# kdsuneraavinash/CH-Bin

Hardware: NVIDIA B200
Metric: point-to-hull QP distances/sec (higher is better)
Workload: dtype f64

## Files before the change

### ch-bin_b200/csrc/fused.cu

```cuda
#include <cuda.h>

#include <algorithm>
#include <cmath>
#include <cstdlib>

#include "common.cuh"

namespace {

constexpr int BM = 128, BN = 128, BK = 32;
constexpr int UMMA_K = 8;
constexpr uint32_t TILE_BYTES = BM * BK * 4;
constexpr int FUSED_THREADS = 320;
constexpr int EPI_THREADS = 256;
constexpr uint32_t TMEM_COLS = 256;
constexpr int MAX_BOX = 10;
constexpr int SMEM_LIMIT = 232448;
constexpr int DMAX_F = CHB_FUSED_RESIDENT_DMAX;
constexpr int DMAX_W = 1024;
constexpr int NKT_STREAMED = -1;
constexpr int WIDE_STAGE_BOXES = 4;

constexpr int NC = 16;
struct SmemTail {
    alignas(16) float cand_val[NC][EPI_THREADS];
    alignas(8) uint64_t full_bar[8];
    alignas(8) uint64_t empty_bar[8];
    alignas(8) uint64_t tmem_full_bar[2];
    alignas(8) uint64_t tmem_empty_bar[2];
    alignas(8) uint64_t a_full_bar;
    alignas(8) uint64_t a_empty_bar;
    alignas(8) uint2 prog[MAX_BOX * 8];
    int prog_start[MAX_BOX + 1];
    uint32_t tmem_base;
};

__device__ __forceinline__ uint32_t smem_u32(const void *p) { return (uint32_t)__cvta_generic_to_shared(p); }
__device__ __forceinline__ void st_shared_f32(uint32_t addr, float v) { asm volatile("st.shared.f32 [%0], %1;" ::"r"(addr), "f"(v) : "memory"); }
__device__ __forceinline__ float ld_shared_f32(uint32_t addr)
{
    float v;
    asm volatile("ld.shared.f32 %0, [%1];" : "=f"(v) : "r"(addr) : "memory");
    return v;
}
__device__ __forceinline__ void mbar_init(uint64_t *bar, uint32_t count)
{
    asm volatile("mbarrier.init.shared::cta.b64 [%0], %1;" ::"r"(smem_u32(bar)), "r"(count));
}
__device__ __forceinline__ void mbar_expect_tx(uint64_t *bar, uint32_t bytes)
{
    asm volatile("mbarrier.arrive.expect_tx.shared::cta.b64 _, [%0], %1;" ::"r"(smem_u32(bar)), "r"(bytes) : "memory");
}
__device__ __forceinline__ void mbar_arrive(uint64_t *bar)
{
    asm volatile("mbarrier.arrive.shared::cta.b64 _, [%0];" ::"r"(smem_u32(bar)) : "memory");
}
__device__ __forceinline__ void mbar_wait(uint64_t *bar, uint32_t parity)
{
    asm volatile(
        "{\n"
        ".reg .pred p;\n"
        "WAIT_LOOP:\n"
        "mbarrier.try_wait.parity.shared::cta.b64 p, [%0], %1;\n"
        "@p bra WAIT_DONE;\n"
        "bra WAIT_LOOP;\n"
        "WAIT_DONE:\n"
        "}\n" ::"r"(smem_u32(bar)),
        "r"(parity)
        : "memory");
}
__device__ __forceinline__ void tma_load_2d(void *smem_dst, const CUtensorMap *map, uint64_t *bar, int c0, int c1)
{
    asm volatile("cp.async.bulk.tensor.2d.shared::cluster.global.mbarrier::complete_tx::bytes [%0], [%1, {%3, %4}], [%2];"
                 ::"r"(smem_u32(smem_dst)), "l"(map), "r"(smem_u32(bar)), "r"(c0), "r"(c1)
                 : "memory");
}
__device__ __forceinline__ void umma_tf32(uint32_t tmem_d, uint64_t adesc, uint64_t bdesc, uint32_t idesc, uint32_t accumulate)
{
    asm volatile(
        "{\n"
        ".reg .pred p;\n"
        "setp.ne.b32 p, %4, 0;\n"
        "tcgen05.mma.cta_group::1.kind::tf32 [%0], %1, %2, %3, p;\n"
        "}\n" ::"r"(tmem_d),
        "l"(adesc), "l"(bdesc), "r"(idesc), "r"(accumulate)
        : "memory");
}
__device__ __forceinline__ bool elect_one_sync()
{
    uint32_t pred;
    asm volatile(
        "{\n"
        ".reg .pred P;\n"
        "elect.sync _|P, 0xffffffff;\n"
        "selp.b32 %0, 1, 0, P;\n"
        "}\n"
        : "=r"(pred));
    return pred != 0;
}
__device__ __forceinline__ void umma_commit(uint64_t *bar)
{
    asm volatile("tcgen05.commit.cta_group::1.mbarrier::arrive::one.shared::cluster.b64 [%0];" ::"r"(smem_u32(bar)) : "memory");
}

__global__ void round_reset_kernel(int32_t *__restrict__ bin_cnt, int32_t nbin_cnt, float *__restrict__ ym2, int32_t nym2,
                                   int32_t *__restrict__ row_nb, int64_t nown, int32_t *__restrict__ pair_meta, int32_t nmeta,
                                   int32_t *__restrict__ pair_row, int64_t cap_pairs, int32_t *__restrict__ counters,
                                   int64_t ncol, int32_t *__restrict__ col_pt, int32_t *__restrict__ col_a, int32_t *__restrict__ col_b)
{
    chb_pdl_enter();
    const int64_t i = (int64_t)blockIdx.x * blockDim.x + threadIdx.x;
    if (i < ncol) {
        col_pt[i] = -1;
        col_a[i] = INT32_MAX;
        col_b[i] = INT32_MIN;
    }
    if (i < nbin_cnt) bin_cnt[i] = 0;
    if (i < nym2) ym2[i] = 0.f;
    if (i < nown) row_nb[i] = 0;
    if (i < nmeta) pair_meta[i] = 0;
    if (i < cap_pairs) pair_row[i] = -1;
    if (i == 0) {
        counters[0] = 0; counters[6] = 0; counters[7] = 0; counters[8] = 0; counters[12] = 0; counters[14] = 0;
        counters[1] = 0x7f7f7f7f; counters[2] = 0; counters[3] = 0;
    }
}
// ... 760 lines not shown
            const int v = beg[b];
            nxt = v > nxt ? nxt : v;
            beg[b] = nxt;
        }
        totals[0] = TT;
    }
    if (beg_smem) {
        __syncthreads();
        for (int b = tid; b <= G; b += 1024) cta_begin[b] = s_begin[b];
    }
}

template <bool WIDE>
__global__ void __launch_bounds__(256) pairs_fill_kernel(const int32_t *__restrict__ mode, const int32_t *__restrict__ row_nb,
                                                         const int32_t *__restrict__ row_bins, int64_t nown, int32_t C,
                                                         const int32_t *__restrict__ pair_off, int32_t *__restrict__ pair_row,
                                                         int32_t *__restrict__ row_pid, const float *__restrict__ a2, int32_t Kp2,
                                                         float *__restrict__ ap)
{
    chb_pdl_enter();
    if (*mode != 1) return;
    const int lane = threadIdx.x & 31;
    const int64_t r = ((int64_t)blockIdx.x * blockDim.x + threadIdx.x) >> 5;
    if (r >= nown) return;
    const int nb = row_nb[r];
    if (nb == 0) return;
    const float4 *src = reinterpret_cast<const float4 *>(a2 + r * Kp2);
    const int nq = Kp2 / 4;
    float4 v[3];
    if constexpr (!WIDE) {
#pragma unroll
        for (int u = 0; u < 3; ++u) v[u] = (lane + 32 * u < nq) ? __ldg(src + lane + 32 * u) : make_float4(0.f, 0.f, 0.f, 0.f);
    }
    for (int jb = 0; jb < nb; jb += 32) {
        const int j = jb + lane;
        int id = -1;
        if (j < nb) {
            const int c = row_bins[r * C + j];
            id = pair_off[c] + row_pid[r * C + j];
            pair_row[id] = (int32_t)r;
            row_pid[r * C + j] = id;
        }
        const int cnt = nb - jb < 32 ? nb - jb : 32;
        for (int w = 0; w < cnt; ++w) {
            const int idw = __shfl_sync(CHB_FULL, id, w);
            float4 *dst = reinterpret_cast<float4 *>(ap + (int64_t)idw * Kp2);
            if constexpr (WIDE) {
                for (int u = lane; u < nq; u += 32) dst[u] = __ldg(src + u);
            } else {
#pragma unroll
                for (int u = 0; u < 3; ++u)
                    if (lane + 32 * u < nq) dst[lane + 32 * u] = v[u];
            }
        }
    }
}

template <int KR>
struct TopList {
    float key[KR];
    int idx[KR];
    __device__ __forceinline__ void reset()
    {
#pragma unroll
        for (int s = 0; s < KR; ++s) { key[s] = INFINITY; idx[s] = INT32_MAX; }
    }
    __device__ __forceinline__ void insert(float ka, int ki)
    {
        int cnt = 0;
#pragma unroll
        for (int s = 0; s < KR; ++s) cnt += (key[s] <= ka) ? 1 : 0;
#pragma unroll
        for (int s = KR - 1; s >= 1; --s) {
            const bool shift = s > cnt, here = s == cnt;
            key[s] = shift ? key[s - 1] : (here ? ka : key[s]);
            idx[s] = shift ? idx[s - 1] : (here ? ki : idx[s]);
        }
        key[0] = cnt == 0 ? ka : key[0];
        idx[0] = cnt == 0 ? ki : idx[0];
    }
};

template <int KR, int NKT>
__global__ void __launch_bounds__(FUSED_THREADS, 1)
gram_select_kernel(const __grid_constant__ CUtensorMap map_a, const __grid_constant__ CUtensorMap map_ap,
                   const __grid_constant__ CUtensorMap map_b, const int32_t *__restrict__ mode_p,
                   const int32_t *__restrict__ pair_row, int nbox, int nk, int nstage,
                   const int32_t *__restrict__ col_pt,
                   const int32_t *__restrict__ col_a, const int32_t *__restrict__ col_b, const float *__restrict__ col_nrm,
                   const float *__restrict__ tq_tab, const int32_t *__restrict__ row_point, const int32_t *__restrict__ pos,
                   int64_t nrows, int32_t C, const float *__restrict__ t0_tab, int64_t ldt, const int4 *__restrict__ items,
                   const int32_t *__restrict__ cta_begin, float *__restrict__ cand_key, int32_t *__restrict__ cand_idx,
                   int32_t *__restrict__ tiles_issued)
{
    chb_pdl_wait();
    const int item_begin = cta_begin[blockIdx.x], item_end = cta_begin[blockIdx.x + 1];
    const int mode = *mode_p;
    constexpr bool STREAM = NKT == NKT_STREAMED;
    constexpr uint32_t STAGE_BYTES = STREAM ? WIDE_STAGE_BOXES * TILE_BYTES : TILE_BYTES;
    extern __shared__ uint8_t smem_raw[];
    uint8_t *base = reinterpret_cast<uint8_t *>((reinterpret_cast<uintptr_t>(smem_raw) + 1023) & ~uintptr_t(1023));
    uint8_t *a_res = base;
    uint8_t *ring = STREAM ? base : base + (size_t)nbox * TILE_BYTES;
    SmemTail &S = *reinterpret_cast<SmemTail *>(ring + (size_t)nstage * STAGE_BYTES);
    const int warp = threadIdx.x >> 5, lane = threadIdx.x & 31;

    if (threadIdx.x == 0) {
        for (int s = 0; s < nstage; ++s) {
            mbar_init(&S.full_bar[s], 1);
            mbar_init(&S.empty_bar[s], 1);
        }
        for (int b = 0; b < 2; ++b) {
            mbar_init(&S.tmem_full_bar[b], 1);
            mbar_init(&S.tmem_empty_bar[b], 8);
        }
        mbar_init(&S.a_full_bar, 1);
        mbar_init(&S.a_empty_bar, 1);
        asm volatile("fence.mbarrier_init.release.cluster;" ::: "memory");
        asm volatile("prefetch.tensormap [%0];" ::"l"(&map_a) : "memory");
        asm volatile("prefetch.tensormap [%0];" ::"l"(&map_ap) : "memory");
        asm volatile("prefetch.tensormap [%0];" ::"l"(&map_b) : "memory");
    }
    if (warp == 2) {
        asm volatile("tcgen05.alloc.cta_group::1.sync.aligned.shared::cta.b32 [%0], %1;" ::"r"(smem_u32(&S.tmem_base)), "n"(TMEM_COLS));
        asm volatile("tcgen05.relinquish_alloc_permit.cta_group::1.sync.aligned;");
    }
    asm volatile("tcgen05.fence::before_thread_sync;" ::: "memory");
    __syncthreads();
    asm volatile("tcgen05.fence::after_thread_sync;" ::: "memory");
    const uint32_t tmem_base = S.tmem_base;

    if (warp == 0) {
        if (lane == 0) {
            int s = 0;
            uint32_t ph = 0;
            int cur_rb = -1, na = 0;
            for (int it = item_begin; it < item_end; ++it) {
                const int4 item = items[it];
                if constexpr (STREAM) {
                    const int H = nbox >> 1;
                    const CUtensorMap *mq = mode ? &map_ap : &map_a;
                    for (int t = item.z; t < item.z + item.w; ++t) {
                        for (int b = 0; b < H; ++b) {
                            uint8_t *st = ring + (size_t)s * STAGE_BYTES;
                            mbar_wait(&S.empty_bar[s], ph ^ 1);
                            mbar_expect_tx(&S.full_bar[s], STAGE_BYTES);
                            tma_load_2d(st, mq, &S.full_bar[s], b * BK, item.x * BM);
                            tma_load_2d(st + TILE_BYTES, mq, &S.full_bar[s], (H + b) * BK, item.x * BM);
                            tma_load_2d(st + 2 * TILE_BYTES, &map_b, &S.full_bar[s], b * BK, t * BN);
                            tma_load_2d(st + 3 * TILE_BYTES, &map_b, &S.full_bar[s], (H + b) * BK, t * BN);
                            if (++s == nstage) { s = 0; ph ^= 1; }
                        }
                    }
                    continue;
                }
                if (item.x != cur_rb) {
                    mbar_wait(&S.a_empty_bar, (uint32_t)((na & 1) ^ 1));
                    mbar_expect_tx(&S.a_full_bar, (uint32_t)nbox * TILE_BYTES);
                    for (int jb = 0; jb < nbox; ++jb)
                        tma_load_2d(a_res + (size_t)jb * TILE_BYTES, mode ? &map_ap : &map_a, &S.a_full_bar, jb * BK, item.x * BM);
                    cur_rb = item.x;
                    ++na;
                }
                for (int t = item.z; t < item.z + item.w; ++t) {
                    for (int jb = 0; jb < nbox; ++jb) {
                        mbar_wait(&S.empty_bar[s], ph ^ 1);
                        mbar_expect_tx(&S.full_bar[s], TILE_BYTES);
                        tma_load_2d(ring + (size_t)s * TILE_BYTES, &map_b, &S.full_bar[s], jb * BK, t * BN);
                        if (++s == nstage) { s = 0; ph ^= 1; }
                    }
                }
            }
        }
    } else if (warp == 1) {
        {
            const uint32_t idesc = (1u << 4) | (2u << 7) | (2u << 10) | ((uint32_t)(BN >> 3) << 17) | ((uint32_t)(BM >> 4) << 24);
            const uint32_t a_addr = smem_u32(a_res);
            constexpr uint32_t DESC_HI = (1024u >> 4) | (1u << 14) | (2u << 29);
            if (NKT == 0 && lane == 0) {
                int m = 0;
                for (int jb = 0; jb < nbox; ++jb) {
                    S.prog_start[jb] = m;
                    for (int u = 0; u < BK / UMMA_K; ++u) {
                        const int j = jb * (BK / UMMA_K) + u;
                        if (j >= 2 * nk) break;
                        const int i0 = j < nk ? j : j - nk;
                        const uint32_t boff = (uint32_t)((u * UMMA_K * 4) >> 4);
                        S.prog[m++] = make_uint2((((a_addr + (uint32_t)(i0 >> 2) * TILE_BYTES) & 0x3FFFFu) >> 4 | (1u << 16)) +
                                                     (uint32_t)(((i0 & 3) * UMMA_K * 4) >> 4), boff);
                        if (j < nk) {
                            const int i1 = nk + j;
                            S.prog[m++] = make_uint2((((a_addr + (uint32_t)(i1 >> 2) * TILE_BYTES) & 0x3FFFFu) >> 4 | (1u << 16)) +
                                                         (uint32_t)(((i1 & 3) * UMMA_K * 4) >> 4), boff);
                        }
                    }
                }
                S.prog_start[nbox] = m;
            }
            __syncwarp();
            const uint32_t ring_lo = ((smem_u32(ring) & 0x3FFFFu) >> 4) | (1u << 16);
            int s = 0;
            uint32_t ph = 0;
            int64_t tt = 0;
            int cur_rb = -1, na = 0;
            for (int it = item_begin; it < item_end; ++it) {
                const int4 item = items[it];
                if (!STREAM && item.x != cur_rb) {
                    if (cur_rb >= 0 && elect_one_sync()) umma_commit(&S.a_empty_bar);
                    mbar_wait(&S.a_full_bar, (uint32_t)(na & 1));
                    asm volatile("tcgen05.fence::after_thread_sync;" ::: "memory");
                    cur_rb = item.x;
                    ++na;
                }
                for (int t = item.z; t < item.z + item.w; ++t) {
                    const int buf = (int)(tt & 1);
                    const uint32_t tph = (uint32_t)((tt >> 1) & 1);
                    ++tt;
                    mbar_wait(&S.tmem_empty_bar[buf], tph ^ 1);
                    asm volatile("tcgen05.fence::after_thread_sync;" ::: "memory");
                    const uint32_t tmem_d = tmem_base + (uint32_t)(buf * BN);
                    if constexpr (STREAM) {
                        const int H = nbox >> 1;
                        for (int b = 0; b < H; ++b) {
                            const uint32_t st_lo = ring_lo + (uint32_t)s * (STAGE_BYTES >> 4);
                            mbar_wait(&S.full_bar[s], ph);
                            asm volatile("tcgen05.fence::after_thread_sync;" ::: "memory");
                            if (elect_one_sync()) {
#pragma unroll
                                for (int u = 0; u < BK / UMMA_K; ++u) {
                                    const uint32_t ko = (uint32_t)((u * UMMA_K * 4) >> 4);
                                    const uint64_t qhi = ((uint64_t)DESC_HI << 32) | (st_lo + ko);
                                    const uint64_t qlo = ((uint64_t)DESC_HI << 32) | (st_lo + (TILE_BYTES >> 4) + ko);
                                    const uint64_t chi = ((uint64_t)DESC_HI << 32) | (st_lo + 2 * (TILE_BYTES >> 4) + ko);
                                    const uint64_t clo = ((uint64_t)DESC_HI << 32) | (st_lo + 3 * (TILE_BYTES >> 4) + ko);
                                    umma_tf32(tmem_d, qhi, chi, idesc, (b | u) != 0);
                                    umma_tf32(tmem_d, qlo, chi, idesc, 1u);
                                    umma_tf32(tmem_d, qhi, clo, idesc, 1u);
                                }
                                umma_commit(&S.empty_bar[s]);
                            }
                            if (++s == nstage) { s = 0; ph ^= 1; }
                        }
                    } else if constexpr (NKT > 0) {
                        constexpr int NBOX = (2 * NKT + 3) / 4;
                        const uint32_t a_lo = ((a_addr & 0x3FFFFu) >> 4) | (1u << 16);
#pragma unroll
                        for (int jb = 0; jb < NBOX; ++jb) {
                            const uint32_t b_lo = ring_lo + (uint32_t)s * (TILE_BYTES >> 4);
                            mbar_wait(&S.full_bar[s], ph);
                            asm volatile("tcgen05.fence::after_thread_sync;" ::: "memory");
                            if (elect_one_sync()) {
#pragma unroll
                            for (int u = 0; u < BK / UMMA_K; ++u) {
                                const int j = jb * (BK / UMMA_K) + u;
                                if (j < 2 * NKT) {
                                    const int i0 = j < NKT ? j : j - NKT;
                                    const uint64_t bdesc = ((uint64_t)DESC_HI << 32) | (b_lo + (uint32_t)((u * UMMA_K * 4) >> 4));
                                    umma_tf32(tmem_d,
                                              ((uint64_t)DESC_HI << 32) |
                                                  (a_lo + (uint32_t)((i0 >> 2) * (TILE_BYTES >> 4) + (((i0 & 3) * UMMA_K * 4) >> 4))),
                                              bdesc, idesc, (jb | u) != 0);
                                    if (j < NKT) {
                                        const int i1 = NKT + j;
                                        umma_tf32(tmem_d,
                                                  ((uint64_t)DESC_HI << 32) |
                                                      (a_lo + (uint32_t)((i1 >> 2) * (TILE_BYTES >> 4) + (((i1 & 3) * UMMA_K * 4) >> 4))),
                                                  bdesc, idesc, 1u);
                                    }
                                }
                            }
                            umma_commit(&S.empty_bar[s]);
                            }
                            if (++s == nstage) { s = 0; ph ^= 1; }
                        }
                    } else {
                        uint32_t acc = 0;
                        int m = 0;
                        for (int jb = 0; jb < nbox; ++jb) {
                            const int m_end = S.prog_start[jb + 1];
                            const uint32_t b_lo = ring_lo + (uint32_t)s * (TILE_BYTES >> 4);
                            mbar_wait(&S.full_bar[s], ph);
                            asm volatile("tcgen05.fence::after_thread_sync;" ::: "memory");
                            if (elect_one_sync()) {
                                for (int mm = m; mm < m_end; ++mm) {
                                    const uint2 e = S.prog[mm];
                                    const uint64_t adesc = ((uint64_t)DESC_HI << 32) | e.x;
                                    const uint64_t bdesc = ((uint64_t)DESC_HI << 32) | (b_lo + e.y);
                                    umma_tf32(tmem_d, adesc, bdesc, idesc, (mm | (int)acc) != 0);
                                }
                                umma_commit(&S.empty_bar[s]);
                            }
                            m = m_end;
                            acc = 1;
                            if (++s == nstage) { s = 0; ph ^= 1; }
                        }
                    }
                    if (elect_one_sync()) umma_commit(&S.tmem_full_bar[buf]);
                }
            }
            if (lane == 0 && tt > 0) atomicAdd(tiles_issued, (int32_t)tt);
        }
    } else {
        const int q = warp & 3;
        const int half = (warp - 2) >> 2;
        const int row = q * 32 + lane;
        const int et = threadIdx.x - 64;
        TopList<KR> L;
        int64_t tt = 0;
        const uint32_t cand_base = smem_u32(&S.cand_val[0][et]);
        for (int it = item_begin; it < item_end; ++it) {
            const int4 item = items[it];
            const int cur_bin = item.y;
            const int64_t gid = (int64_t)item.x * BM + row;
            const int64_t gr = mode ? (int64_t)pair_row[gid] : gid;
            const bool rvalid = gr >= 0 && gr < nrows;
            const int p = rvalid ? pos[row_point[gr]] : INT32_MIN + 1;
            const float t0 = rvalid ? t0_tab[(int64_t)cur_bin * ldt + gr] : -INFINITY;
            const float nr = rvalid ? tq_tab[(int64_t)cur_bin * ldt + gr] : 0.f;
            L.reset();
            const bool wskip = __all_sync(CHB_FULL, !(t0 > -INFINITY));
            for (int t = item.z; t < item.z + item.w; ++t) {
                const int buf = (int)(tt & 1);
                const uint32_t tph = (uint32_t)((tt >> 1) & 1);
                ++tt;
                if (wskip) {
                    mbar_wait(&S.tmem_full_bar[buf], tph);
                    asm volatile("tcgen05.fence::after_thread_sync;" ::: "memory");
                    asm volatile("tcgen05.fence::before_thread_sync;" ::: "memory");
                    __syncwarp();
                    if (lane == 0) mbar_arrive(&S.tmem_empty_bar[buf]);
                    continue;
                }
                if (lane < 6 && (t + 1 < item.z + item.w || it + 1 < item_end)) {
                    const int tn = t + 1 < item.z + item.w ? t + 1 : items[it + 1].z;
                    const int64_t e = (int64_t)tn * BN + half * 64 + (lane & 1) * 32;
                    const void *pf = lane < 2 ? (const void *)(col_nrm + e) : (lane < 4 ? (const void *)(col_a + e) : (const void *)(col_b + e));
                    asm volatile("prefetch.global.L1 [%0];" ::"l"(pf));
                }
                const int64_t e0 = (int64_t)t * BN + half * 64;
                const float4 *mn = reinterpret_cast<const float4 *>(col_nrm + e0);
                const int4 *ma = reinterpret_cast<const int4 *>(col_a + e0);
                const int4 *mb = reinterpret_cast<const int4 *>(col_b + e0);
                const int32_t *tile_pt = col_pt + e0;
                mbar_wait(&S.tmem_full_bar[buf], tph);
                asm volatile("tcgen05.fence::after_thread_sync;" ::: "memory");
                uint32_t v[64];
                {
                    const uint32_t taddr = tmem_base + ((uint32_t)(q * 32) << 16) + (uint32_t)(buf * BN + half * 64);
                    asm volatile("tcgen05.ld.sync.aligned.32x32b.x64.b32 {%0, %1, %2, %3, %4, %5, %6, %7, %8, %9, %10, %11, %12, %13, %14, %15, %16, %17, %18, %19, %20, %21, %22, %23, %24, %25, %26, %27, %28, %29, %30, %31, %32, %33, %34, %35, %36, %37, %38, %39, %40, %41, %42, %43, %44, %45, %46, %47, %48, %49, %50, %51, %52, %53, %54, %55, %56, %57, %58, %59, %60, %61, %62, %63}, [%64];"
                                 : "=r"(v[0]), "=r"(v[1]), "=r"(v[2]), "=r"(v[3]), "=r"(v[4]), "=r"(v[5]), "=r"(v[6]), "=r"(v[7]), "=r"(v[8]), "=r"(v[9]), "=r"(v[10]), "=r"(v[11]), "=r"(v[12]), "=r"(v[13]), "=r"(v[14]), "=r"(v[15]), "=r"(v[16]), "=r"(v[17]), "=r"(v[18]), "=r"(v[19]), "=r"(v[20]), "=r"(v[21]), "=r"(v[22]), "=r"(v[23]), "=r"(v[24]), "=r"(v[25]), "=r"(v[26]), "=r"(v[27]), "=r"(v[28]), "=r"(v[29]), "=r"(v[30]), "=r"(v[31]), "=r"(v[32]), "=r"(v[33]), "=r"(v[34]), "=r"(v[35]), "=r"(v[36]), "=r"(v[37]), "=r"(v[38]), "=r"(v[39]), "=r"(v[40]), "=r"(v[41]), "=r"(v[42]), "=r"(v[43]), "=r"(v[44]), "=r"(v[45]), "=r"(v[46]), "=r"(v[47]), "=r"(v[48]), "=r"(v[49]), "=r"(v[50]), "=r"(v[51]), "=r"(v[52]), "=r"(v[53]), "=r"(v[54]), "=r"(v[55]), "=r"(v[56]), "=r"(v[57]), "=r"(v[58]), "=r"(v[59]), "=r"(v[60]), "=r"(v[61]), "=r"(v[62]), "=r"(v[63])
                                 : "r"(taddr));
                    asm volatile("tcgen05.wait::ld.sync.aligned;" ::: "memory");
                    asm volatile("tcgen05.fence::before_thread_sync;" ::: "memory");
                    __syncwarp();
                    if (lane == 0) mbar_arrive(&S.tmem_empty_bar[buf]);
                }
                int ncand = 0;
                unsigned cm_lo = 0, cm_hi = 0;
                int g = 0;
#define SCREEN_STEP(G)                                                                                              \
    case G: {                                                                                                       \
        const float thr = fminf(L.key[KR - 1], t0);                                                                 \
        const float4 n4 = __ldg(mn + G);                                                                            \
        const int4 a4 = __ldg(ma + G);                                                                              \
        const int4 b4 = __ldg(mb + G);                                                                              \
        const float nn[4] = {n4.x, n4.y, n4.z, n4.w};                                                               \
        const int aa[4] = {a4.x, a4.y, a4.z, a4.w};                                                                 \
        const int bb[4] = {b4.x, b4.y, b4.z, b4.w};                                                                 \
        _Pragma("unroll") for (int u = 0; u < 4; ++u) {                                                             \
            const float av = fmaf(-2.f, __uint_as_float(v[4 * G + u]), nr + nn[u]);                                 \
            if (((p > aa[u]) || (p < bb[u])) && (av <= thr)) {                                                      \
                st_shared_f32(cand_base + (uint32_t)ncand * (EPI_THREADS * 4), av);                                 \
                if (G < 8) cm_lo |= 1u << ((4 * G + u) & 31);                                                       \
                else cm_hi |= 1u << ((4 * G + u) & 31);                                                             \
                ++ncand;                                                                                            \
            }                                                                                                       \
        }                                                                                                           \
        if (G < 15 && __any_sync(CHB_FULL, ncand > NC - 4)) {                                                       \
            g = G + 1;                                                                                              \
            break;                                                                                                  \
        }                                                                                                           \
    }
                while (true) {
                    switch (g) {
                    SCREEN_STEP(0)
                    SCREEN_STEP(1)
                    SCREEN_STEP(2)
                    SCREEN_STEP(3)
                    SCREEN_STEP(4)
                    SCREEN_STEP(5)
                    SCREEN_STEP(6)
                    SCREEN_STEP(7)
                    SCREEN_STEP(8)
                    SCREEN_STEP(9)
                    SCREEN_STEP(10)
                    SCREEN_STEP(11)
                    SCREEN_STEP(12)
                    SCREEN_STEP(13)
                    SCREEN_STEP(14)
                    SCREEN_STEP(15)
                        g = 16;
                    }
                    while (__any_sync(CHB_FULL, ncand > 0)) {
                        if (ncand > 0) {
                            --ncand;
                            int col;
                            if (cm_hi) { col = 63 - __clz(cm_hi); cm_hi &= ~(1u << (col - 32)); }
                            else { col = 31 - __clz(cm_lo); cm_lo &= ~(1u << col); }
                            const float av = ld_shared_f32(cand_base + (uint32_t)ncand * (EPI_THREADS * 4));
                            if (av < L.key[KR - 1]) L.insert(av, __ldg(tile_pt + col));
                        }
                    }
                    if (g >= 16) break;
                }
#undef SCREEN_STEP
            }
            if (rvalid && !wskip) {
                const int64_t lslot = mode ? gid : gr * C + cur_bin;
                float4 *ok = reinterpret_cast<float4 *>(cand_key + (lslot * 2 + half) * KR);
                int4 *oi = reinterpret_cast<int4 *>(cand_idx + (lslot * 2 + half) * KR);
#pragma unroll
                for (int s = 0; s < KR; s += 4) {
                    ok[s >> 2] = make_float4(L.key[s], L.key[s + 1], L.key[s + 2], L.key[s + 3]);
                    oi[s >> 2] = make_int4(L.idx[s], L.idx[s + 1], L.idx[s + 2], L.idx[s + 3]);
                }
            }
        }
    }
    asm volatile("tcgen05.fence::before_thread_sync;" ::: "memory");
    __syncthreads();
    if (warp == 2) {
        asm volatile("tcgen05.dealloc.cta_group::1.sync.aligned.b32 %0, %1;" ::"r"(tmem_base), "n"(TMEM_COLS));
    }
}

constexpr int THR_BINS = 4;
template <int THR_ROWS>
__global__ void __launch_bounds__(256) threshold_kernel(const int32_t *__restrict__ knn_idx, const int32_t *__restrict__ knn_cnt, const float *__restrict__ thr,
                                 const int32_t *__restrict__ row_point, const int32_t *__restrict__ row_slot,
                                 const int32_t *__restrict__ pos, const int32_t *__restrict__ tent, const int32_t *__restrict__ old,
                                 const float *__restrict__ nrm, const unsigned int *__restrict__ nrm_max_bits,
                                 const float *__restrict__ ym2, const float *__restrict__ tcmax, const float *__restrict__ tq_tab,
                                 const float *__restrict__ ub_row, const float *__restrict__ sq_row,
                                 const float *__restrict__ ubk2_row, const int32_t *__restrict__ row_guess, double eps_rel, int64_t nown,
                                 int32_t C, int32_t k, int32_t prune, int64_t ldt, float *__restrict__ t0_tab, float *__restrict__ slack_tab,
                                 int32_t *__restrict__ row_nb, int32_t *__restrict__ row_bins, int32_t *__restrict__ bin_surv,
                                 uint8_t *__restrict__ skip, int32_t *__restrict__ row_pid)
{
    chb_pdl_enter();
    constexpr int NBIN = THR_ROWS == 4 ? THR_BINS : 1;
    const int lane = threadIdx.x & 31;
    const int64_t r0 = ((int64_t)blockIdx.x * 256 + threadIdx.x) * THR_ROWS;
    float4 tq4s[NBIN], ub4 = make_float4(0.f, 0.f, 0.f, 0.f), sq4 = ub4;
    if (THR_ROWS == 4 && r0 < nown) {
        ub4 = *reinterpret_cast<const float4 *>(ub_row + r0);
        sq4 = *reinterpret_cast<const float4 *>(sq_row + r0);
#pragma unroll
        for (int cb = 0; cb < NBIN; ++cb) {
            const int cc = blockIdx.y * NBIN + cb;
            tq4s[cb] = cc < C ? *reinterpret_cast<const float4 *>(tq_tab + (int64_t)cc * ldt + r0) : ub4;
        }
    }
#pragma unroll
    for (int cb = 0; cb < NBIN; ++cb) {
    const int c = blockIdx.y * NBIN + cb;
    if (c >= C) break;
    bool any_alive = false;
    if (r0 < nown) {
        float tqv[4], ubv[4], sqv[4];
        if (THR_ROWS == 4) {
            const float4 tq4 = tq4s[cb];
            tqv[0] = tq4.x; tqv[1] = tq4.y; tqv[2] = tq4.z; tqv[3] = tq4.w;
            ubv[0] = ub4.x; ubv[1] = ub4.y; ubv[2] = ub4.z; ubv[3] = ub4.w;
            sqv[0] = sq4.x; sqv[1] = sq4.y; sqv[2] = sq4.z; sqv[3] = sq4.w;
        } else {
            tqv[0] = tq_tab[(int64_t)c * ldt + r0];
            ubv[0] = ub_row[r0];
            sqv[0] = sq_row[r0];
        }
        const float ym = __fmul_ru(__fsqrt_ru(ym2[c]), 1.000001f), amax = __fsqrt_ru(__uint_as_float(*nrm_max_bits));
        float t0v[4] = {-INFINITY, -INFINITY, -INFINITY, -INFINITY};
        bool alive[4] = {false, false, false, false};
#pragma unroll
        for (int u = 0; u < THR_ROWS; ++u) {
            alive[u] = r0 + u < nown;
            t0v[u] = -INFINITY;
            if (alive[u] && prune) {
                const float dq = __fsqrt_rd(tqv[u]), ub = ubv[u];
                const float scale = sqv[u] + amax;
                if (dq * 0.999999f - ym > ub + 1e-5f * (dq + ym + ub) + 4e-6f * scale) alive[u] = false;
            }
            any_alive = any_alive || alive[u];
        }
        if (any_alive) {
#pragma unroll
            for (int u = 0; u < THR_ROWS; ++u) {
                if (!alive[u]) continue;
                const int64_t r = r0 + u;
                const float tq = tqv[u];
                const int js = atomicAdd(&row_nb[r], 1);
                row_bins[r * C + js] = c;
// ... 598 lines not shown
            for (int t = 0; t < m; ++t) rk += I[t] < my ? 1 : 0;
            __syncwarp();
            if (lane < m) srt[rk] = my;
            __syncwarp();
            const int64_t pair = (int64_t)row_slot[r] * C + c;
            const bool diff = lane < k && knn_idx[pair * k + lane] != (lane < m ? srt[lane] : -1);
            const bool same = knn_cnt[pair] == m && !__any_sync(CHB_FULL, diff);
            if (!same) {
                if (lane < k) knn_idx[pair * k + lane] = lane < m ? srt[lane] : -1;
                if (lane == 0) {
                    knn_cnt[pair] = m;
                    work[atomicAdd(work_count, 1)] = make_int2(row_slot[r], c);
                }
            }
        }
    }
}

typedef CUresult (*encode_fn_t)(CUtensorMap *, CUtensorMapDataType, cuuint32_t, void *, const cuuint64_t *, const cuuint64_t *,
                                const cuuint32_t *, const cuuint32_t *, CUtensorMapInterleave, CUtensorMapSwizzle,
                                CUtensorMapL2promotion, CUtensorMapFloatOOBfill);
encode_fn_t get_encode_fn()
{
    static encode_fn_t fn = nullptr;
    if (!fn) {
        void *p = nullptr;
        cudaDriverEntryPointQueryResult qres;
        if (cudaGetDriverEntryPoint("cuTensorMapEncodeTiled", &p, cudaEnableDefault, &qres) == cudaSuccess &&
            qres == cudaDriverEntryPointSuccess)
            fn = reinterpret_cast<encode_fn_t>(p);
    }
    return fn;
}
int make_map(chb_ctx *ctx, CUtensorMap *map, float *base, int64_t nrows, int32_t Kp)
{
    encode_fn_t enc = get_encode_fn();
    CHB_CHECK(ctx, enc != nullptr, CHB_ECUDA, "cuTensorMapEncodeTiled entry point not available");
    const cuuint64_t gdim[2] = {(cuuint64_t)Kp, (cuuint64_t)nrows};
    const cuuint64_t gstr[1] = {(cuuint64_t)Kp * sizeof(float)};
    const cuuint32_t box[2] = {(cuuint32_t)BK, (cuuint32_t)BM};
    const cuuint32_t estr[2] = {1, 1};
    CUresult r = enc(map, CU_TENSOR_MAP_DATA_TYPE_FLOAT32, 2, base, gdim, gstr, box, estr, CU_TENSOR_MAP_INTERLEAVE_NONE,
                     CU_TENSOR_MAP_SWIZZLE_128B, CU_TENSOR_MAP_L2_PROMOTION_L2_256B, CU_TENSOR_MAP_FLOAT_OOB_FILL_NONE);
    CHB_CHECK(ctx, r == CUDA_SUCCESS, CHB_ECUDA, "cuTensorMapEncodeTiled failed (%d)", (int)r);
    return CHB_OK;
}

struct FusedGeom {
    int dp8, nk, nbox, Kp2, nstage;
    bool stream;
    size_t smem;
};
FusedGeom fused_geom(int d)
{
    FusedGeom g{};
    const int fixed = 1024 + (int)sizeof(SmemTail);
    g.stream = d > DMAX_F;
    if (g.stream) {
        g.dp8 = (d + BK - 1) & ~(BK - 1);
        g.nk = g.dp8 / UMMA_K;
        g.nbox = 2 * g.dp8 / BK;
        g.Kp2 = g.nbox * BK;
        const int stage = WIDE_STAGE_BOXES * (int)TILE_BYTES;
        g.nstage = std::min(8, (SMEM_LIMIT - fixed) / stage);
        g.smem = (size_t)fixed + (size_t)g.nstage * stage;
        return g;
    }
    g.dp8 = (d + 7) & ~7;
    g.nk = g.dp8 / UMMA_K;
    g.nbox = (2 * g.dp8 + BK - 1) / BK;
    g.Kp2 = g.nbox * BK;
    g.nstage = std::min(8, (SMEM_LIMIT - fixed - g.nbox * (int)TILE_BYTES) / (int)TILE_BYTES);
    g.smem = (size_t)fixed + (size_t)(g.nbox + std::max(g.nstage, 0)) * TILE_BYTES;
    return g;
}

template <int KR, int NKT>
int launch_fused(chb_ctx *c, const CUtensorMap &ma, const CUtensorMap &map, const CUtensorMap &mb, int64_t nrows, const FusedGeom &g)
{
    CHB_CUDA(c, cudaFuncSetAttribute(gram_select_kernel<KR, NKT>, cudaFuncAttributeMaxDynamicSharedMemorySize, (int)g.smem));
    const int grid = c->sm_count;
    {
        chb_stage_timer t(c, CHB_ST_GRAM);
        CHB_PDL_LAUNCH(c, (gram_select_kernel<KR, NKT>), grid, FUSED_THREADS, g.smem,
            ma, map, mb, c->f_mode, c->f_pair_row, g.nbox, g.nk, g.nstage, c->f_col_pt, c->f_col_a, c->f_col_b, c->f_col_nrm, c->f_tq, c->f_row_pt, c->pos, nrows, c->C,
            c->f_t0, c->f_ldt, c->f_items, c->f_cta_begin, c->f_cand_key, c->f_cand_idx, &c->counters[8]);
    }
    CHB_CUDA(c, cudaGetLastError());
    return CHB_OK;
}

template <int KR>
int dispatch_nk(chb_ctx *c, const CUtensorMap &ma, const CUtensorMap &map, const CUtensorMap &mb, int64_t nrows, const FusedGeom &g)
{
    if (g.stream) return launch_fused<KR, NKT_STREAMED>(c, ma, map, mb, nrows, g);
    const bool generic = getenv("CHB_FUSED_GENERIC") != nullptr;
    if (!generic && g.nk == 18) return launch_fused<KR, 18>(c, ma, map, mb, nrows, g);
    if (!generic && g.nk == 19) return launch_fused<KR, 19>(c, ma, map, mb, nrows, g);
    if (!generic && g.nk == 20) return launch_fused<KR, 20>(c, ma, map, mb, nrows, g);
    return launch_fused<KR, 0>(c, ma, map, mb, nrows, g);
}
int dispatch_fused(chb_ctx *c, const CUtensorMap &ma, const CUtensorMap &map, const CUtensorMap &mb, int64_t nrows, const FusedGeom &g,
                   int KR)
{
    return KR == 8 ? dispatch_nk<8>(c, ma, map, mb, nrows, g) : dispatch_nk<16>(c, ma, map, mb, nrows, g);
}

template <typename T>
int reserve(chb_ctx *ctx, T **p, int64_t *cap, int64_t count)
{
    if (*p && *cap >= count) return CHB_OK;
    if (*p) cudaFree(*p);
    *p = nullptr;
    *cap = 0;
    cudaError_t e = cudaMalloc(reinterpret_cast<void **>(p), sizeof(T) * (size_t)std::max<int64_t>(count, 1));
    if (e != cudaSuccess) {
        (void)cudaGetLastError();
        return chb_fail(ctx, CHB_ENOMEM, "cudaMalloc of %lld bytes failed: %s", (long long)(sizeof(T) * (size_t)count),
                        cudaGetErrorString(e));
    }
    *cap = count;
    return CHB_OK;
}

inline unsigned nblk(int64_t n, int t) { return (unsigned)((n + t - 1) / t); }

}

bool chb_fused_supported(const chb_ctx *c)
{
    const FusedGeom g = fused_geom(c->d);
    if (c->k > XS_KEEP || c->d > DMAX_W) return false;
    return g.nstage >= 3 && (g.stream || g.nbox <= MAX_BOX);
}

void chb_fused_free(chb_ctx *c)
{
    if (c->side_stream) cudaStreamSynchronize(c->side_stream);
    c->side_join_pending = false;
    cudaFree(c->f_bin_cnt); cudaFree(c->f_seg_off); cudaFree(c->f_cursor); cudaFree(c->f_tile_bin); cudaFree(c->f_ntiles);
    cudaFree(c->f_col_pt); cudaFree(c->f_col_a); cudaFree(c->f_col_b); cudaFree(c->f_col_nrm); cudaFree(c->f_bperm);
    cudaFree(c->f_cand_key); cudaFree(c->f_cand_idx); cudaFree(c->f_fb_pairs); cudaFree(c->f_xs_slots); cudaFree(c->f_thr); cudaFree(c->f_t0); cudaFree(c->f_a2); cudaFree(c->f_tq); cudaFree(c->f_slack); cudaFree(c->f_ym2);
    cudaFree(c->f_mc); cudaFree(c->f_mc2); cudaFree(c->f_mcnt); cudaFree(c->f_skip); cudaFree(c->f_pair_row); cudaFree(c->f_pair_meta); cudaFree(c->f_ap); cudaFree(c->f_mode); cudaFree(c->f_items); cudaFree(c->f_cta_begin); cudaFree(c->f_row_slot); cudaFree(c->f_row_pt);
    cudaFree(c->f_ub); cudaFree(c->f_ubk2); cudaFree(c->f_row_guess); cudaFree(c->f_rhist); cudaFree(c->f_mcT); cudaFree(c->f_guess_all); cudaFree(c->f_tqs);
    c->f_tqs = nullptr;
    c->f_cap_tqs = 0; cudaFree(c->f_seedT); cudaFree(c->f_row_nb); cudaFree(c->f_row_bins); cudaFree(c->f_row_pid); cudaFree(c->f_slot_row); cudaFree(c->f_sq_row);
    c->f_slot_row = nullptr;
    c->f_sq_row = nullptr;
    c->f_seedT = nullptr;
    c->f_row_nb = c->f_row_bins = c->f_row_pid = nullptr;
    c->f_cap_seedT = 0;
    c->f_mcT = nullptr;
    c->f_guess_all = nullptr;
    c->f_cap_guess = c->f_cap_mcT = 0;
    c->f_skip = nullptr;
    c->f_pair_row = c->f_pair_meta = c->f_mode = nullptr;
    c->f_ap = nullptr;
    c->f_cap_ap = c->f_cap_pairs = 0;
    c->f_items = nullptr;
    c->f_cta_begin = nullptr;
    c->f_row_slot = c->f_row_pt = nullptr;
    c->f_ub = c->f_ubk2 = nullptr;
    c->f_row_guess = c->f_rhist = nullptr;
    c->f_thr = c->f_t0 = c->f_a2 = c->f_tq = c->f_slack = c->f_ym2 = nullptr;
    c->f_mc = c->f_mc2 = nullptr;
    c->f_mcnt = nullptr;
    c->f_cap_mc = 0;
// ... 443 lines not shown
```

Measured before the change: 2.582 billion.

## Double epilogue warps for KR=8 and quadruple TMEM accumulator buffers

For KR=8 the epilogue grows from 8 to 16 warps, so each warp screens 32 columns of a tile instead of 64. The two lists that cover the same half are then merged through shared memory with named barriers. The TMEM accumulator ring grows from 2 to 4 buffers (512 columns), letting the MMA warp run further ahead of the epilogue. The aim is to lift the epilogue's selection throughput, which bounds the kernel. The cost is a larger block, an extra merge with three barrier syncs per item, and more TMEM allocation.

```diff
diff --git a/ch-bin_b200/csrc/fused.cu b/ch-bin_b200/csrc/fused.cu
--- a/ch-bin_b200/csrc/fused.cu
+++ b/ch-bin_b200/csrc/fused.cu
@@ -11,9 +11,10 @@
 constexpr int BM = 128, BN = 128, BK = 32;
 constexpr int UMMA_K = 8;
 constexpr uint32_t TILE_BYTES = BM * BK * 4;
-constexpr int FUSED_THREADS = 320;
-constexpr int EPI_THREADS = 256;
-constexpr uint32_t TMEM_COLS = 256;
+__host__ __device__ constexpr int epi_warps(int KR) { return KR == 8 ? 16 : 8; }
+__host__ __device__ constexpr int fused_threads(int KR) { return 64 + 32 * epi_warps(KR); }
+constexpr int NACC = 4;
+constexpr uint32_t TMEM_COLS = NACC * 128;
 constexpr int MAX_BOX = 10;
 constexpr int SMEM_LIMIT = 232448;
 constexpr int DMAX_F = CHB_FUSED_RESIDENT_DMAX;
@@ -21,19 +22,20 @@
 constexpr int NKT_STREAMED = -1;
 constexpr int WIDE_STAGE_BOXES = 4;
 
-constexpr int NC = 16;
+constexpr int CAND_WORDS = 16 * 256;
 struct SmemTail {
-    alignas(16) float cand_val[NC][EPI_THREADS];
+    alignas(16) float cand_val[CAND_WORDS];
     alignas(8) uint64_t full_bar[8];
     alignas(8) uint64_t empty_bar[8];
-    alignas(8) uint64_t tmem_full_bar[2];
-    alignas(8) uint64_t tmem_empty_bar[2];
+    alignas(8) uint64_t tmem_full_bar[NACC];
+    alignas(8) uint64_t tmem_empty_bar[NACC];
     alignas(8) uint64_t a_full_bar;
     alignas(8) uint64_t a_empty_bar;
     alignas(8) uint2 prog[MAX_BOX * 8];
     int prog_start[MAX_BOX + 1];
     uint32_t tmem_base;
 };
+static_assert(1024 + sizeof(SmemTail) + 13 * TILE_BYTES <= SMEM_LIMIT, "SmemTail costs a ring stage");
 
 __device__ __forceinline__ uint32_t smem_u32(const void *p) { return (uint32_t)__cvta_generic_to_shared(p); }
 __device__ __forceinline__ void st_shared_f32(uint32_t addr, float v) { asm volatile("st.shared.f32 [%0], %1;" ::"r"(addr), "f"(v) : "memory"); }
@@ -42,6 +44,10 @@
     float v;
     asm volatile("ld.shared.f32 %0, [%1];" : "=f"(v) : "r"(addr) : "memory");
     return v;
+}
+__device__ __forceinline__ void named_bar_sync(uint32_t id, uint32_t nthreads)
+{
+    asm volatile("bar.sync %0, %1;" ::"r"(id), "r"(nthreads) : "memory");
 }
 __device__ __forceinline__ void mbar_init(uint64_t *bar, uint32_t count)
 {
@@ -968,7 +974,7 @@
 };
 
 template <int KR, int NKT>
-__global__ void __launch_bounds__(FUSED_THREADS, 1)
+__global__ void __launch_bounds__(fused_threads(KR), 1)
 gram_select_kernel(const __grid_constant__ CUtensorMap map_a, const __grid_constant__ CUtensorMap map_ap,
                    const __grid_constant__ CUtensorMap map_b, const int32_t *__restrict__ mode_p,
                    const int32_t *__restrict__ pair_row, int nbox, int nk, int nstage,
@@ -996,9 +1002,9 @@
             mbar_init(&S.full_bar[s], 1);
             mbar_init(&S.empty_bar[s], 1);
         }
-        for (int b = 0; b < 2; ++b) {
+        for (int b = 0; b < NACC; ++b) {
             mbar_init(&S.tmem_full_bar[b], 1);
-            mbar_init(&S.tmem_empty_bar[b], 8);
+            mbar_init(&S.tmem_empty_bar[b], epi_warps(KR));
         }
         mbar_init(&S.a_full_bar, 1);
         mbar_init(&S.a_empty_bar, 1);
@@ -1099,8 +1105,8 @@
                     ++na;
                 }
                 for (int t = item.z; t < item.z + item.w; ++t) {
-                    const int buf = (int)(tt & 1);
-                    const uint32_t tph = (uint32_t)((tt >> 1) & 1);
+                    const int buf = (int)(tt % NACC);
+                    const uint32_t tph = (uint32_t)((tt / NACC) & 1);
                     ++tt;
                     mbar_wait(&S.tmem_empty_bar[buf], tph ^ 1);
                     asm volatile("tcgen05.fence::after_thread_sync;" ::: "memory");
@@ -1187,13 +1193,20 @@
             if (lane == 0 && tt > 0) atomicAdd(tiles_issued, (int32_t)tt);
         }
     } else {
+        constexpr int EPI_T = 32 * epi_warps(KR);
+        constexpr int COLS = 4 * BN / epi_warps(KR);
+        constexpr int NG = COLS / 4;
+        constexpr int NC = CAND_WORDS / EPI_T;
+        static_assert(COLS == 32 || COLS == 64, "epilogue layout");
+        static_assert(COLS == 64 || KR <= NC, "a quarter-list must fit one candidate stack for the merge");
         const int q = warp & 3;
-        const int half = (warp - 2) >> 2;
+        const int part = (warp - 2) >> 2;
+        const int half = part * COLS / 64;
         const int row = q * 32 + lane;
         const int et = threadIdx.x - 64;
         TopList<KR> L;
         int64_t tt = 0;
-        const uint32_t cand_base = smem_u32(&S.cand_val[0][et]);
+        const uint32_t cand_base = smem_u32(&S.cand_val[et]);
         for (int it = item_begin; it < item_end; ++it) {
             const int4 item = items[it];
             const int cur_bin = item.y;
@@ -1203,11 +1216,12 @@
             const int p = rvalid ? pos[row_point[gr]] : INT32_MIN + 1;
             const float t0 = rvalid ? t0_tab[(int64_t)cur_bin * ldt + gr] : -INFINITY;
             const float nr = rvalid ? tq_tab[(int64_t)cur_bin * ldt + gr] : 0.f;
+            const int64_t lslot = mode ? gid : gr * C + cur_bin;
             L.reset();
             const bool wskip = __all_sync(CHB_FULL, !(t0 > -INFINITY));
             for (int t = item.z; t < item.z + item.w; ++t) {
-                const int buf = (int)(tt & 1);
-                const uint32_t tph = (uint32_t)((tt >> 1) & 1);
+                const int buf = (int)(tt % NACC);
+                const uint32_t tph = (uint32_t)((tt / NACC) & 1);
                 ++tt;
                 if (wskip) {
                     mbar_wait(&S.tmem_full_bar[buf], tph);
@@ -1217,22 +1231,28 @@
                     if (lane == 0) mbar_arrive(&S.tmem_empty_bar[buf]);
                     continue;
                 }
-                if (lane < 6 && (t + 1 < item.z + item.w || it + 1 < item_end)) {
+                constexpr int LPA = COLS / 32;
+                if (lane < 3 * LPA && (t + 1 < item.z + item.w || it + 1 < item_end)) {
                     const int tn = t + 1 < item.z + item.w ? t + 1 : items[it + 1].z;
-                    const int64_t e = (int64_t)tn * BN + half * 64 + (lane & 1) * 32;
-                    const void *pf = lane < 2 ? (const void *)(col_nrm + e) : (lane < 4 ? (const void *)(col_a + e) : (const void *)(col_b + e));
+                    const int64_t e = (int64_t)tn * BN + part * COLS + (lane % LPA) * 32;
+                    const void *pf = lane < LPA ? (const void *)(col_nrm + e) : (lane < 2 * LPA ? (const void *)(col_a + e) : (const void *)(col_b + e));
                     asm volatile("prefetch.global.L1 [%0];" ::"l"(pf));
                 }
-                const int64_t e0 = (int64_t)t * BN + half * 64;
+                const int64_t e0 = (int64_t)t * BN + part * COLS;
                 const float4 *mn = reinterpret_cast<const float4 *>(col_nrm + e0);
                 const int4 *ma = reinterpret_cast<const int4 *>(col_a + e0);
                 const int4 *mb = reinterpret_cast<const int4 *>(col_b + e0);
                 const int32_t *tile_pt = col_pt + e0;
                 mbar_wait(&S.tmem_full_bar[buf], tph);
                 asm volatile("tcgen05.fence::after_thread_sync;" ::: "memory");
-                uint32_t v[64];
+                uint32_t v[COLS];
                 {
-                    const uint32_t taddr = tmem_base + ((uint32_t)(q * 32) << 16) + (uint32_t)(buf * BN + half * 64);
+                    const uint32_t taddr = tmem_base + ((uint32_t)(q * 32) << 16) + (uint32_t)(buf * BN + part * COLS);
+                    if constexpr (COLS == 32)
+                    asm volatile("tcgen05.ld.sync.aligned.32x32b.x32.b32 {%0, %1, %2, %3, %4, %5, %6, %7, %8, %9, %10, %11, %12, %13, %14, %15, %16, %17, %18, %19, %20, %21, %22, %23, %24, %25, %26, %27, %28, %29, %30, %31}, [%32];"
+                                 : "=r"(v[0]), "=r"(v[1]), "=r"(v[2]), "=r"(v[3]), "=r"(v[4]), "=r"(v[5]), "=r"(v[6]), "=r"(v[7]), "=r"(v[8]), "=r"(v[9]), "=r"(v[10]), "=r"(v[11]), "=r"(v[12]), "=r"(v[13]), "=r"(v[14]), "=r"(v[15]), "=r"(v[16]), "=r"(v[17]), "=r"(v[18]), "=r"(v[19]), "=r"(v[20]), "=r"(v[21]), "=r"(v[22]), "=r"(v[23]), "=r"(v[24]), "=r"(v[25]), "=r"(v[26]), "=r"(v[27]), "=r"(v[28]), "=r"(v[29]), "=r"(v[30]), "=r"(v[31])
+                                 : "r"(taddr));
+                    else
                     asm volatile("tcgen05.ld.sync.aligned.32x32b.x64.b32 {%0, %1, %2, %3, %4, %5, %6, %7, %8, %9, %10, %11, %12, %13, %14, %15, %16, %17, %18, %19, %20, %21, %22, %23, %24, %25, %26, %27, %28, %29, %30, %31, %32, %33, %34, %35, %36, %37, %38, %39, %40, %41, %42, %43, %44, %45, %46, %47, %48, %49, %50, %51, %52, %53, %54, %55, %56, %57, %58, %59, %60, %61, %62, %63}, [%64];"
                                  : "=r"(v[0]), "=r"(v[1]), "=r"(v[2]), "=r"(v[3]), "=r"(v[4]), "=r"(v[5]), "=r"(v[6]), "=r"(v[7]), "=r"(v[8]), "=r"(v[9]), "=r"(v[10]), "=r"(v[11]), "=r"(v[12]), "=r"(v[13]), "=r"(v[14]), "=r"(v[15]), "=r"(v[16]), "=r"(v[17]), "=r"(v[18]), "=r"(v[19]), "=r"(v[20]), "=r"(v[21]), "=r"(v[22]), "=r"(v[23]), "=r"(v[24]), "=r"(v[25]), "=r"(v[26]), "=r"(v[27]), "=r"(v[28]), "=r"(v[29]), "=r"(v[30]), "=r"(v[31]), "=r"(v[32]), "=r"(v[33]), "=r"(v[34]), "=r"(v[35]), "=r"(v[36]), "=r"(v[37]), "=r"(v[38]), "=r"(v[39]), "=r"(v[40]), "=r"(v[41]), "=r"(v[42]), "=r"(v[43]), "=r"(v[44]), "=r"(v[45]), "=r"(v[46]), "=r"(v[47]), "=r"(v[48]), "=r"(v[49]), "=r"(v[50]), "=r"(v[51]), "=r"(v[52]), "=r"(v[53]), "=r"(v[54]), "=r"(v[55]), "=r"(v[56]), "=r"(v[57]), "=r"(v[58]), "=r"(v[59]), "=r"(v[60]), "=r"(v[61]), "=r"(v[62]), "=r"(v[63])
                                  : "r"(taddr));
@@ -1245,7 +1265,7 @@
                 unsigned cm_lo = 0, cm_hi = 0;
                 int g = 0;
 #define SCREEN_STEP(G)                                                                                              \
-    case G: {                                                                                                       \
+    case G: if constexpr (G < NG) {                                                                                 \
         const float thr = fminf(L.key[KR - 1], t0);                                                                 \
         const float4 n4 = __ldg(mn + G);                                                                            \
         const int4 a4 = __ldg(ma + G);                                                                              \
@@ -1256,13 +1276,13 @@
         _Pragma("unroll") for (int u = 0; u < 4; ++u) {                                                             \
             const float av = fmaf(-2.f, __uint_as_float(v[4 * G + u]), nr + nn[u]);                                 \
             if (((p > aa[u]) || (p < bb[u])) && (av <= thr)) {                                                      \
-                st_shared_f32(cand_base + (uint32_t)ncand * (EPI_THREADS * 4), av);                                 \
+                st_shared_f32(cand_base + (uint32_t)ncand * (EPI_T * 4), av);                                       \
                 if (G < 8) cm_lo |= 1u << ((4 * G + u) & 31);                                                       \
                 else cm_hi |= 1u << ((4 * G + u) & 31);                                                             \
                 ++ncand;                                                                                            \
             }                                                                                                       \
         }                                                                                                           \
-        if (G < 15 && __any_sync(CHB_FULL, ncand > NC - 4)) {                                                       \
+        if (G < NG - 1 && __any_sync(CHB_FULL, ncand > NC - 4)) {                                                   \
             g = G + 1;                                                                                              \
             break;                                                                                                  \
         }                                                                                                           \
@@ -1285,7 +1305,7 @@
                     SCREEN_STEP(13)
                     SCREEN_STEP(14)
                     SCREEN_STEP(15)
-                        g = 16;
+                        g = NG;
                     }
                     while (__any_sync(CHB_FULL, ncand > 0)) {
                         if (ncand > 0) {
@@ -1293,16 +1313,47 @@
                             int col;
                             if (cm_hi) { col = 63 - __clz(cm_hi); cm_hi &= ~(1u << (col - 32)); }
                             else { col = 31 - __clz(cm_lo); cm_lo &= ~(1u << col); }
-                            const float av = ld_shared_f32(cand_base + (uint32_t)ncand * (EPI_THREADS * 4));
+                            const float av = ld_shared_f32(cand_base + (uint32_t)ncand * (EPI_T * 4));
                             if (av < L.key[KR - 1]) L.insert(av, __ldg(tile_pt + col));
                         }
                     }
-                    if (g >= 16) break;
+                    if (g >= NG) break;
                 }
 #undef SCREEN_STEP
             }
-            if (rvalid && !wskip) {
-                const int64_t lslot = mode ? gid : gr * C + cur_bin;
+            const bool writer = COLS == 64 || (part & 1) == 0;
+            if constexpr (COLS == 32) {
+                if (!wskip) {
+                    const uint32_t bar = 1 + (uint32_t)(half * 4 + q);
+                    const uint32_t key_col = (part & 1) ? cand_base : cand_base + 128 * 4;
+                    const uint32_t idx_col = key_col - 128 * 4;
+                    named_bar_sync(bar, 64);
+                    if (!writer) {
+#pragma unroll
+                        for (int s = 0; s < KR; ++s) {
+                            st_shared_f32(key_col + (uint32_t)s * (EPI_T * 4), L.key[s]);
+                            st_shared_f32(idx_col + (uint32_t)s * (EPI_T * 4), __int_as_float(L.idx[s]));
+                        }
+                    }
+                    named_bar_sync(bar, 64);
+                    float ok[KR];
+                    int oi[KR];
+                    if (writer) {
+#pragma unroll
+                        for (int s = 0; s < KR; ++s) {
+                            ok[s] = ld_shared_f32(key_col + (uint32_t)s * (EPI_T * 4));
+                            oi[s] = __float_as_int(ld_shared_f32(idx_col + (uint32_t)s * (EPI_T * 4)));
+                        }
+                    }
+                    named_bar_sync(bar, 64);
+                    if (writer) {
+#pragma unroll
+                        for (int s = 0; s < KR; ++s)
+                            if (ok[s] < L.key[KR - 1]) L.insert(ok[s], oi[s]);
+                    }
+                }
+            }
+            if (writer && rvalid && !wskip) {
                 float4 *ok = reinterpret_cast<float4 *>(cand_key + (lslot * 2 + half) * KR);
                 int4 *oi = reinterpret_cast<int4 *>(cand_idx + (lslot * 2 + half) * KR);
 #pragma unroll
@@ -2067,7 +2118,7 @@
     const int grid = c->sm_count;
     {
         chb_stage_timer t(c, CHB_ST_GRAM);
-        CHB_PDL_LAUNCH(c, (gram_select_kernel<KR, NKT>), grid, FUSED_THREADS, g.smem,
+        CHB_PDL_LAUNCH(c, (gram_select_kernel<KR, NKT>), grid, fused_threads(KR), g.smem,
             ma, map, mb, c->f_mode, c->f_pair_row, g.nbox, g.nk, g.nstage, c->f_col_pt, c->f_col_a, c->f_col_b, c->f_col_nrm, c->f_tq, c->f_row_pt, c->pos, nrows, c->C,
             c->f_t0, c->f_ldt, c->f_items, c->f_cta_begin, c->f_cand_key, c->f_cand_idx, &c->counters[8]);
     }
```

Result: faster. 2.650 billion, median of 6 (+2.6%).
